# tuffy/flac-codec

Hardware: AMD Instinct MI355X
Metric: Msamples/s encode at level 8, 48kHz/24-bit stereo; bit-exact vs reference (higher is better)
Workload: dtype i32/i64 (+f64 LPC analysis); 1 GPU; config 3: 48 kHz/24-bit stereo, blocksize 4096, level 8 (Options::best: LPC order 12, partition order 6, mid-side, exhaustive); 8192 frames per GPU per step, PCM resident in HBM, frame bytes produc...; level=L8, frames_per_gpu=8192, contexts=3, parallelism=frame ranges x1

## Files before the change

flac-codec_amd/csrc/autocorr.hip:

```cpp
#include "kernels/types.h"

#include <stdlib.h>

#include <type_traits>

namespace {
#include "kernels/common.inc"
#include "kernels/lpc.inc"
#include "kernels/autocorr.inc"

template <int NL, bool STEREO>
bool launch_autocorr3(const Params &p, uint32_t frame0, uint32_t nframes, uint32_t n, const double *win, hipStream_t st) {
    const uint32_t groups = (nframes * p.ncand + 63) / 64;
    if constexpr (STEREO) {
        if (p.inter) {
            if (groups <= 64 && NL == 13)
                hipLaunchKernelGGL(HIP_KERNEL_NAME(k_autocorr4<13, 8, true, true, 0, true>), dim3(groups), dim3(512), 0, st, p,
                                   frame0, nframes, n, win);
            else
                hipLaunchKernelGGL(HIP_KERNEL_NAME(k_autocorr4<NL, 4, true, true, 0, true>), dim3(groups), dim3(256), 0, st, p,
                                   frame0, nframes, n, win);
            return true;
        }
    }
    if constexpr (!STEREO) {
        if (p.split_src) {
#define AC4_SPLIT(C)                                                                                                      \
    hipLaunchKernelGGL(HIP_KERNEL_NAME(k_autocorr4<NL, 4, false, true, C, true>), dim3(groups), dim3(256), 0, st, p, frame0, \
                       nframes, n, win)
            if (p.channels == 8) AC4_SPLIT(8);
            else if (p.channels == 4) AC4_SPLIT(4);
            else AC4_SPLIT(0);
#undef AC4_SPLIT
            return true;
        }
    }
    if (p.ac_split == 2)
        hipLaunchKernelGGL(HIP_KERNEL_NAME(k_autocorr4<NL, 2, STEREO>), dim3(groups), dim3(128), 0, st, p,
                           frame0, nframes, n, win);
    else
        hipLaunchKernelGGL(HIP_KERNEL_NAME(k_autocorr4<NL, 4, STEREO>), dim3(groups), dim3(256), 0, st, p,
                           frame0, nframes, n, win);
    return false;
}
template <bool STEREO>
bool launch_autocorr3_nl(const Params &p, uint32_t frame0, uint32_t nframes, uint32_t n, const double *win, hipStream_t st) {
    const uint32_t nl = p.max_lpc_order + 1;
    if (nl <= 5) return launch_autocorr3<5, STEREO>(p, frame0, nframes, n, win, st);
    if (nl <= 9) return launch_autocorr3<9, STEREO>(p, frame0, nframes, n, win, st);
    if (nl <= 13) return launch_autocorr3<13, STEREO>(p, frame0, nframes, n, win, st);
    return launch_autocorr3<17, STEREO>(p, frame0, nframes, n, win, st);
}
bool try_autocorr3(const Params &p, uint32_t frame0, uint32_t nframes, uint32_t n, const double *win, hipStream_t st,
                   bool *fused) {
    *fused = false;
    if (n < 32 || n % 32 != 0) return false;
    const bool stereo = p.stereo4 && p.ncand == 4 && p.channels == 2 && p.bps <= 24;
    const bool indep = !p.stereo4 && p.ncand == p.channels;
    if (!stereo && !indep) return false;
    if (p.max_lpc_order > 16) {
        if (n % 64 != 0) return false;
        const uint32_t groups = (nframes * p.ncand + 63) / 64;
        if (stereo && p.inter) {
            hipLaunchKernelGGL(HIP_KERNEL_NAME(k_autocorr4_deep<true, true>), dim3(groups), dim3(256), 0, st, p, frame0,
                               nframes, n, win);
        } else if (stereo) {
            hipLaunchKernelGGL(HIP_KERNEL_NAME(k_autocorr4_deep<true>), dim3(groups), dim3(256), 0, st, p, frame0,
                               nframes, n, win);
// ... 61 lines not shown
```

flac-codec_amd/csrc/flacenc_gpu.hip:

```cpp
#include "kernels/types.h"
#include "kernels/place_rule.h"
#include "batch_route.h"
#include "lpc_host.h"
#include "ragged_plan.h"

#include <ctype.h>
#include <math.h>
#include <stdint.h>
#include <stdio.h>
#include <stdlib.h>
#include <string.h>

#include <algorithm>
#include <atomic>
#include <cmath>
#include <chrono>
#include <functional>
#include <mutex>
#include <thread>
#include <string>
#include <type_traits>
#include <vector>

thread_local std::string g_last_error;

static std::atomic<uint64_t> g_early_downloads{0}, g_early_remainders{0};
extern "C" void flacgpu_early_download_counters(uint64_t *queued, uint64_t *with_remainder) {
    if (queued) *queued = g_early_downloads.load();
    if (with_remainder) *with_remainder = g_early_remainders.load();
}
static constexpr uint32_t kDeferMargin16 = 48;
static constexpr uint32_t kDeferWords = DEFER_SLOTS * DEFER_SLOT_WORDS;
static constexpr uint32_t kTurnWords = 4;
Knobs read_knobs() {
    Knobs k;
    auto on = [](const char *name) { return getenv(name) != nullptr; };
    k.no_direct = on("FLACGPU_NO_DIRECT");
    k.no_cand_pair = on("FLACGPU_NO_CAND_PAIR");
    k.force_fir_check = on("FLACGPU_FIR_CHECK");
    k.no_xpose = on("FLACGPU_NO_XPOSE");
    k.no_ac_fma = on("FLACGPU_NO_AC_FMA");
    k.no_hand = on("FLACGPU_NO_HAND");
    k.no_direct_short = on("FLACGPU_NO_DIRECT_SHORT");
    k.no_ragged = on("FLACGPU_NO_RAGGED");
    k.no_w64 = on("FLACGPU_NO_W64");
    k.no_fused_pack = on("FLACGPU_NO_FUSED_PACK");
    k.no_frame64 = on("FLACGPU_NO_FRAME64");
    k.early_download = on("FLACGPU_EARLY_DOWNLOAD");
    if (const char *e = getenv("FLACGPU_CAND_GRID")) k.cand_grid = (uint32_t)atoi(e);
    if (const char *e = getenv("FLACGPU_DEFER_FIXED")) k.defer_fixed = atoi(e);
    if (const char *e = getenv("FLACGPU_DEFER_MARGIN16")) k.defer_margin16 = atoi(e);
    const char *t = getenv("FLACGPU_TEST_KNOBS");
    if (t && t[0] == '1') {
        k.experiment_mfma_ac = on("FLACGPU_EXPERIMENT_MFMA_AC");
        if (const char *e = getenv("FLACGPU_TIE_BAND")) { k.has_tie_band = true; k.tie_band = atof(e); }
        if (const char *e = getenv("FLACGPU_TIE_PERTURB")) { k.has_tie_perturb = true; k.tie_perturb = atof(e); }
        if (const char *e = getenv("FLACGPU_FIR_SUSPECT_BITS")) k.fir_suspect_bits = (uint32_t)atoi(e);
    }
    return k;
}

namespace {
#include "kernels/common.inc"
#include "kernels/k0_split.inc"
#include "kernels/generic_analysis.inc"
#include "kernels/generic_fir.inc"
#include "kernels/decide_emit.inc"
}
using namespace flacgpu_k;
using flacenc_route::Route;
using flacenc_route::RouteBatch;
using flacenc_route::RouteContext;

struct flacgpu_ctx;
static uint32_t *defer_stats_of(const flacgpu_ctx *c);
static int ctx_sync(flacgpu_ctx *c);
static hipStream_t ctx_stream(flacgpu_ctx *c);

struct flacgpu_ctx {
    flacgpu_options opts;
    uint32_t bps, channels, max_frames, ldb, ncand, stereo4;
    int device;
    int32_t *d_in = nullptr, *d_planar = nullptr, *d_resid = nullptr;
    double *d_window_full = nullptr, *d_window_last = nullptr, *d_log2_thr = nullptr, *d_ac = nullptr;
    CandInfo *d_cinfo = nullptr;
    SubPlan *d_fixed = nullptr, *d_cand = nullptr, *d_out = nullptr;
    LpcParams *d_lpc = nullptr;
    FrameInfo *d_finfo = nullptr;
    uint32_t *d_hand = nullptr;
    flacgpu_frame_plan *d_fplan = nullptr;
    uint32_t *d_stats_base = nullptr;
    uint32_t *d_stats = nullptr;
    uint32_t *d_orbits = nullptr;
    uint32_t *d_ties = nullptr;
    double tie_band = 1e-9, tie_perturb = 0.0;
    Knobs knobs;
    uint64_t *d_seg_fn = nullptr, *h_seg = nullptr;
    const int32_t **d_seg_ptr = nullptr;
    std::vector<flacgpu_segment> segs;
    bool seg_pending = false;
    bool seg_active = false;
    bool seg_direct = false;
    uint32_t *d_rag_tab = nullptr, *h_rag_tab = nullptr;
    PlaceRun *d_rag_runs = nullptr, *h_rag_runs = nullptr;
    double *d_rag_pool = nullptr;
    uint64_t rag_pool_cap = 0;
    std::vector<std::pair<uint32_t, uint32_t>> rag_pool_at;
    std::vector<double> rag_pool_host;
    uint64_t rag_pool_uploads = 0;
    std::vector<uint32_t> rag_n;
// ... 599 lines not shown
        } else {
            begin_plain_batch(c);
        }
    }
    const uint32_t B = c->opts.block_size;
    const bool ragged = c->rag_active;
    if (!ragged)
    for (uint32_t n : {n_frames > 1 ? B : last_len, last_len}) {
        uint32_t tz = (uint32_t)__builtin_ctz(n);
        if ((tz < c->opts.max_partition_order ? tz : c->opts.max_partition_order) > (uint32_t)MAXP) {
            g_last_error = "effective partition order > 6: the reference panics (MAX_PARTITIONS = 64)";
            return FLACGPU_ERR_UNSUPPORTED;
        }
    }
    if (!ragged && last_len != B && last_len != c->window_last_len) {
        if (int rc = upload_window(c, last_len, c->d_window_last, st)) return rc;
        c->window_last_len = last_len;
    }
    Params p;
    fill_params(c, n_frames, last_len, p);
    if (ragged) {
        p.frame_n = c->d_rag_tab;
        p.frame_win = c->d_rag_tab + c->max_frames;
        p.window_pool = c->d_rag_pool;
    }
    c->host_out = nullptr;
    c->out_in_host = false;

    int evi = 0;
    for (auto &u : c->ev_used) u = false;
    auto mark = [&](int k) {
        if (c->timing) {
            (void)hipEventRecord(c->ev[evi], st);
            c->ev_used[k] = true;
            evi++;
        }
    };
    int order_of_marks[FLACGPU_N_KERNELS];
    int n_marks = 0;
    auto begin = [&](int k) {
        order_of_marks[n_marks++] = k;
        mark(k);
    };

    const Route r = given ? *given : route_of(c, aligned16(d_pcm), layout, n_frames, last_len, packed_bytes);
    const uint32_t ncb = n_frames * c->ncand;
    const bool ranged = c->rng_cnt != 0;
    const uint32_t rf0 = ranged ? c->rng_f0 : 0u, rcnt = ranged ? c->rng_cnt : n_frames;
    const bool first_range = rf0 == 0;
    if (first_range) HIP_TRY(hipMemsetAsync(c->d_stats_base, 0, sizeof(uint32_t) * (kTurnWords + 4 + (size_t)ncb), st));
    const bool direct = r.input == Route::DIRECT_STEREO, xpose = r.input == Route::SPLIT_XPOSE;
    const bool split = r.input == Route::SPLIT || xpose;
    if (direct) p.inter = d_pcm;
    if (r.hand) p.hand_meta = c->d_hand;
    if (r.segments_in_place) p.inter_tab = c->d_seg_ptr;
    if (split) {
        p.split_src = d_pcm;
        p.split_dst = (c->channels == 1 || xpose) ? nullptr : c->d_planar;
        p.xpose = xpose ? 1u : 0u;
        if (c->channels == 1) p.planar = d_pcm;
    }
    c->abs_valid = false;
    if (c->d_abs && first_range) HIP_TRY(hipMemsetAsync(c->d_abs, 0, sizeof(unsigned long long) * 4 * n_frames, st));
    if (!r.in_place()) begin(0);
    bool have_orbits = true;
    if (r.input == Route::K0_PACKED) {
        launch_k0_packed(c, packed_bytes, n_frames, last_len, st);
    } else if (r.input == Route::PLANAR_IN_PLACE) {
        p.planar = d_pcm;
        have_orbits = false;
    } else if (r.input == Route::K0_COPY) {
        have_orbits = launch_k0(c, d_pcm, layout, n_frames, last_len, 0, n_frames, st);
    }
    if (!have_orbits)
        launch_orbits(p, c->d_orbits, st);
    const size_t dyn2 = (2 * (size_t)B + B / 16 + 16) * sizeof(int32_t);
    if (c->stereo4 && !p.exhaustive && !c->abs_valid && !(direct && p.max_lpc_order == 0)) {
        begin(1);
        if (direct) hipLaunchKernelGGL(k_stereo_stats_t<true>, dim3(n_frames), dim3(WG), 0, st, p);
        else hipLaunchKernelGGL(k_stereo_stats_t<false>, dim3(n_frames), dim3(WG), 0, st, p);
    }
    if (!r.in_place())
        hipLaunchKernelGGL(k_candinfo, dim3((ncb + WG - 1) / WG), dim3(WG), 0, st, p, c->d_orbits,
                           c->abs_valid ? c->d_abs : nullptr);
    Params pf = p, pg = p;
    pf.f0 = rf0;
    pf.fcount = ranged ? rcnt : r.fast_analysis;
    pg.f0 = r.fast_analysis;
    pg.fcount = n_frames - r.fast_analysis;
    const bool lpc = p.max_lpc_order > 0;
    const bool fork = lpc && !c->timing && pg.fcount != 0;
    hipStream_t sf = fork ? c->aux_stream : st;
    if (fork) {
        HIP_TRY(hipEventRecord(c->ev_fork, st));
        HIP_TRY(hipStreamWaitEvent(sf, c->ev_fork, 0));
    }
    if (pg.fcount) {
        begin(2);
        if (B > LDS_BLOCK_LIMIT) hipLaunchKernelGGL(k_fixed_t<true>, dim3(pg.fcount * c->ncand), dim3(WG), 0, sf, pg);
        else hipLaunchKernelGGL(k_fixed_t<false>, dim3(pg.fcount * c->ncand), dim3(WG), dyn2, sf, pg);
    }
    if (fork) HIP_TRY(hipEventRecord(c->ev_join, sf));
    if (lpc) {
        const uint32_t H = ((p.max_lpc_order + 1) + 3u) & ~3u;
        begin(3);
        const uint32_t full = ragged ? 0u : (last_len == B) ? n_frames : n_frames - 1;
// ... 1282 lines not shown
```

flac-codec_amd/csrc/host/batch_route.cpp:

```cpp
#include "batch_route.h"

#include <stddef.h>

namespace flacenc_route {

RouteContext route_context(uint32_t channels, uint32_t bps, uint32_t block_size, uint32_t max_lpc_order,
                           uint32_t max_partition_order, bool exhaustive, const Knobs &knobs) {
    RouteContext c;
    c.channels = channels;
    c.bps = bps;
    c.block_size = block_size;
    c.max_lpc_order = max_lpc_order;
    c.max_partition_order = max_partition_order;
    c.exhaustive = exhaustive;
    c.stereo4 = (channels == 2 && bps < 32) ? 1u : 0u;
    c.ncand = c.stereo4 ? 4u : channels;
    c.has_hand = c.stereo4 && block_size == FN && max_lpc_order > 0 && !knobs.no_hand;
    c.has_edges = channels >= 5;
    c.knobs = knobs;
    return c;
}

namespace {
constexpr int kInterleaved = 0, kPlanar = 1;
constexpr size_t kFrameLdsBytes = 150 * 1024;
bool fits_lds(uint32_t fb_words) { return (size_t)fb_words * sizeof(int32_t) <= kFrameLdsBytes; }
}

Route plan_route(const RouteContext &c, const RouteBatch &b) {
    Route r;
    if (b.ragged) return r;
    const Knobs &kn = c.knobs;
    const uint32_t B = c.block_size, C_ = c.channels, n_frames = b.n_frames;
    const bool whole_blocks = b.last_len == B;
    const uint32_t full = whole_blocks ? n_frames : n_frames - 1;
    const bool narrow = c.bps + (c.stereo4 ? 1u : 0u) <= 25u;
    const bool po_ok = c.max_partition_order <= (uint32_t)MAXP;
    const uint32_t fbw_any = frame_fb_words(C_, c.bps, B);

    const bool w64 = narrow && wave_block_size(B) && (c.max_lpc_order <= 16 || B == FN) && po_ok && !kn.no_w64;
    r.fast_analysis = w64 ? full : 0;

    const uint32_t fbw = (c.stereo4 && c.exhaustive && frame_fb_words_exhaustive_stereo(c.bps, B) < fbw_any)
                             ? frame_fb_words_exhaustive_stereo(c.bps, B) : fbw_any;
    const bool f64w = narrow && wave_block_size(B) && (c.max_lpc_order <= 16 || (B == FN && C_ <= 4)) && (C_ <= 4 || B == FN) &&
                      po_ok && fits_lds(fbw) && !kn.no_fused_pack && !kn.no_frame64;
    r.fast_pack = f64w ? full : 0;
    r.host_out_possible = r.fast_pack != 0 && r.fast_pack == n_frames;
    const bool all_fast = whole_blocks && w64 && f64w;

    const bool in_place_ok = !b.packed_bytes && b.aligned16 && whole_blocks && po_ok && c.lag_split != 2 &&
                             !(kn.no_direct || kn.no_w64 || kn.experiment_mfma_ac);
    const bool direct = in_place_ok && b.layout == kInterleaved && c.stereo4 && C_ == 2 && c.bps <= 24 &&
                        (B == FN || (wave_block_size(B) && c.max_lpc_order <= 16 && !kn.no_direct_short)) &&
                        !kn.no_fused_pack && !kn.no_frame64 && fits_lds(fbw_any);
    const bool planar_rows = !b.packed_bytes && b.aligned16 && (b.layout == kPlanar || C_ == 1) && (B % 4 == 0) && whole_blocks &&
                             !kn.no_direct;
    const bool split = in_place_ok && !c.stereo4 && c.ncand == C_ && c.max_lpc_order >= 1 && c.max_lpc_order <= 16 && B == FN &&
                       c.bps <= 25u && (C_ == 1 ? planar_rows : b.layout == kInterleaved);
    const bool xpose = split && all_fast && !kn.no_xpose && c.bps >= 8 &&
                       (C_ == 3 || C_ == 4 || ((C_ == 8 || C_ == 6) && c.has_edges));
    r.input = direct ? Route::DIRECT_STEREO
              : split ? (xpose ? Route::SPLIT_XPOSE : Route::SPLIT)
              : b.packed_bytes ? Route::K0_PACKED
              : planar_rows ? Route::PLANAR_IN_PLACE
                            : Route::K0_COPY;
    r.hand = direct && B == FN && c.max_lpc_order > 0 && c.has_hand;
    r.segments_in_place = b.segments_in_place_wanted && r.in_place() && C_ >= 2;
    r.k4_in_autocorr = r.in_place() && c.max_lpc_order >= 1 && c.max_lpc_order <= 16;

    if (!b.whole_call || b.packed_bytes || c.timing) return r;
    if (c.two_ranges && n_frames >= 256 && all_fast && fits_lds(fbw_any) && (b.layout == kInterleaved || b.layout == kPlanar)) {
        r.two_ranges = true;
        r.input = (b.layout == kPlanar && planar_rows) ? Route::PLANAR_IN_PLACE : Route::K0_COPY;
        r.hand = r.k4_in_autocorr = r.segments_in_place = false;
        return r;
    }
    if (c.chunk_samples && B == FN && C_ >= 2 && r.in_place() && all_fast && r.k4_in_autocorr &&
        (c.stereo4 ? c.exhaustive : !c.chunk_auto)) {
        const uint32_t chunk = (uint32_t)(c.chunk_samples / ((uint64_t)B * C_)) & ~63u;
        if (chunk >= 256 && n_frames >= chunk + chunk / 2) r.range_frames = chunk;
    }
    return r;
}

}

extern "C" void flacenc_plan_route_row(const int32_t *in, uint32_t *out) {
    using namespace flacenc_route;
    Knobs kn;
    const uint32_t bits = (uint32_t)in[14];
    kn.no_direct = bits & 1u;
    kn.no_w64 = bits & 2u;
    kn.no_fused_pack = bits & 4u;
    kn.no_frame64 = bits & 8u;
    kn.no_direct_short = bits & 16u;
    kn.no_xpose = bits & 32u;
    kn.no_hand = bits & 64u;
    kn.experiment_mfma_ac = bits & 128u;
    RouteContext c = route_context((uint32_t)in[0], (uint32_t)in[1], (uint32_t)in[2], (uint32_t)in[3], (uint32_t)in[4], in[5] != 0, kn);
    c.lag_split = in[11];
    c.timing = in[12] != 0;
    if (in[15] >= 0) {
        c.chunk_samples = chunk_samples_of(in[15]);
        c.chunk_auto = false;
    }
    c.two_ranges = in[16] != 0;
    RouteBatch b;
    b.layout = in[6];
    b.aligned16 = in[7] != 0;
    b.last_len = (uint32_t)in[8];
    b.n_frames = (uint32_t)in[9];
    b.packed_bytes = (uint32_t)in[10];
    b.segments_in_place_wanted = in[13] != 0;
    b.whole_call = in[17] != 0;
    const Route r = plan_route(c, b);
    out[0] = (uint32_t)r.input;
    out[1] = r.hand;
    out[2] = r.fast_analysis;
    out[3] = r.fast_pack;
    out[4] = r.k4_in_autocorr;
    out[5] = r.range_frames;
    out[6] = r.two_ranges;
    out[7] = r.host_out_possible;
    out[8] = r.segments_in_place;
}
```

flac-codec_amd/csrc/host/batch_route.h:

```cpp
#ifndef FLACENC_HOST_BATCH_ROUTE_H
#define FLACENC_HOST_BATCH_ROUTE_H
#include <stdint.h>

#include "../kernels/shape.h"

namespace flacenc_route {

struct RouteContext {
    uint32_t channels = 0, bps = 0, block_size = 0, max_lpc_order = 0, max_partition_order = 0;
    bool exhaustive = false;
    uint32_t stereo4 = 0, ncand = 0;
    bool has_hand = false;
    bool has_edges = false;
    Knobs knobs;
    int lag_split = 4;
    bool two_ranges = false;
    uint32_t chunk_samples = 64u << 20;
    bool chunk_auto = true;
    bool timing = false;
};
inline uint32_t chunk_samples_of(int msamples) { return msamples <= 0 ? 0u : (uint32_t)(msamples < 2047 ? msamples : 2047) << 20; }
RouteContext route_context(uint32_t channels, uint32_t bps, uint32_t block_size, uint32_t max_lpc_order,
                           uint32_t max_partition_order, bool exhaustive, const Knobs &knobs);

struct RouteBatch {
    uint32_t n_frames = 0, last_len = 0;
    int layout = 0;
    bool aligned16 = false;
    uint32_t packed_bytes = 0;
    bool segments_in_place_wanted = false;
    bool whole_call = false;
    bool ragged = false;
};

struct Route {
    enum Input {
        K0_COPY,
        K0_PACKED,
        PLANAR_IN_PLACE,
        DIRECT_STEREO,
        SPLIT,
        SPLIT_XPOSE
    } input = K0_COPY;
    bool hand = false;
    uint32_t fast_analysis = 0;
    uint32_t fast_pack = 0;
    bool k4_in_autocorr = false;
    uint32_t range_frames = 0;
    bool two_ranges = false;
    bool host_out_possible = false;
    bool segments_in_place = false;

    bool in_place() const { return input == DIRECT_STEREO || input == SPLIT || input == SPLIT_XPOSE; }
};

Route plan_route(const RouteContext &c, const RouteBatch &b);

}
#endif
```

flac-codec_amd/csrc/kernels/autocorr.inc:

```


__device__ __forceinline__ void ac4_progress_prio(uint32_t t, uint32_t ntiles) {
    if ((t & 7u) == 0) {
        const uint32_t qd = 4u * t / ntiles;
        if (qd == 0) __builtin_amdgcn_s_setprio(3);
        else if (qd == 1) __builtin_amdgcn_s_setprio(2);
        else if (qd == 2) __builtin_amdgcn_s_setprio(1);
        else __builtin_amdgcn_s_setprio(0);
    }
}

template <int A, int LG, bool FIRST, bool FMA = false>
__device__ __forceinline__ void ac3_block(const double (&w)[16], const double (&prev)[16],
                                          double (&acc)[LG]) {
    if constexpr (FMA) {
        static_assert(!FIRST, "the first block of a frame lies under the window's taper");
#pragma unroll
        for (int s = 0; s < 16; s++) {
#pragma unroll
            for (int k = 0; k < LG; k++) {
                const int lag = A + k;
                const double o = (s - lag >= 0) ? w[(s - lag >= 0) ? s - lag : 0]
                                                : prev[(s - lag >= 0) ? 0 : 16 + s - lag];
                acc[k] = __builtin_fma(w[s], o, acc[k]);
// ... 33 lines not shown
#pragma unroll
            for (int k = 0; k < LG; k++) {
                const int idx = s - (A + k);
                const double o = idx >= 0 ? w[idx >= 0 ? idx : 0]
                               : idx >= -16 ? p1[(idx < 0 && idx >= -16) ? 16 + idx : 0]
                                            : p2[(idx < -16) ? 32 + idx : 0];
                acc[k] = __builtin_fma(w[s], o, acc[k]);
            }
            __builtin_amdgcn_sched_barrier(0);
        }
        return;
    }
#pragma unroll
    for (int s = 0; s < 16; s++) {
        double prod[LG];
#pragma unroll
        for (int k = 0; k < LG; k++) {
            const int idx = s - (A + k);
            const double o = idx >= 0 ? w[idx >= 0 ? idx : 0]
                           : idx >= -16 ? p1[(idx < 0 && idx >= -16) ? 16 + idx : 0]
                                        : p2[(idx < -16) ? 32 + idx : 0];
            prod[k] = w[s] * o;
        }
        __builtin_amdgcn_sched_barrier(0);
#pragma unroll
        for (int k = 0; k < LG; k++) {
            const int lag = A + k;
            if (FIRST == 1 && s < lag) continue;
            if (FIRST == 2 && 16 + s < lag) continue;
            acc[k] = acc[k] + prod[k];
        }
        __builtin_amdgcn_sched_barrier(0);
    }
}

constexpr int AC4_TS = 32;
constexpr int AC4_LDW = AC4_TS + 2;

__device__ __forceinline__ int32_t dpp_row_ror8(int32_t v) {
    int32_t r = __builtin_amdgcn_update_dpp(0, v, 0x128, 0xf, 0xf, false);
    asm volatile("" : "+v"(r));
    return r;
}

template <bool STEREO>
struct Ac4Units {
    static constexpr int PER_TILE = STEREO ? 8 : 16;
    static constexpr int COST = STEREO ? 20 : 10;
};
struct Ac4Share {
    int units[8], first[8];
};
template <bool STEREO>
constexpr Ac4Share ac4_share_n(int ns, const int (&lg)[8]) {
    Ac4Share r{};
    int cost[8] = {};
    for (int w = 0; w < 8; w++) {
        cost[w] = 64 * lg[w];
        r.units[w] = 0;
    }
    for (int u = 0; u < Ac4Units<STEREO>::PER_TILE; u++) {
        int best = 0;
        for (int w = 1; w < ns; w++)
            if (cost[w] < cost[best]) best = w;
        r.units[best]++;
        cost[best] += Ac4Units<STEREO>::COST;
    }
    int f = 0;
    for (int w = 0; w < 8; w++) {
        r.first[w] = f;
        f += r.units[w];
    }
    return r;
}
template <bool STEREO>
constexpr Ac4Share ac4_share(int ns, int lg0, int lg1, int lg2, int lg3) {
    const int lg[8] = {lg0, lg1, lg2, lg3, 0, 0, 0, 0};
    return ac4_share_n<STEREO>(ns, lg);
}

template <int U, bool STEREO>
struct Ac4Producer {
    static constexpr int NU = U > 0 ? U : 1;
    const int32_t *gsrc[NU];
    const double *wsrc[NU];
    uint32_t dst_a[NU], dst_b[NU];
    uint32_t sh_a[NU], sh_b[NU];
    int32_t sgn;
    uint32_t ntiles;
    int2 stage[NU];
    double2 wst[NU];
};

template <int U, int U0, bool STEREO>
__device__ __forceinline__ void ac4_setup(const Params &p, uint32_t frame0, uint32_t nframes, uint32_t n,
                                          const double *__restrict__ win, uint32_t group,
                                          Ac4Producer<U, STEREO> &P) {
    const uint32_t lane = threadIdx.x & 63;
    const uint32_t total = nframes * p.ncand;
    const uint32_t cand0 = group * 64;
    P.ntiles = n / AC4_TS;
    auto wasted_of = [&](uint32_t cc) -> uint32_t {
        const CandInfo ci = p.cinfo[(size_t)frame0 * p.ncand + (cc < total ? cc : total - 1)];
        return (ci.active && !ci.is_const) ? ci.wasted : 0u;
    };
    if constexpr (STEREO) {
        const uint32_t f_lo = cand0 / 4, f_last = nframes - 1;
        const uint32_t is_r = (lane >> 3) & 1u;
        P.sgn = is_r ? -1 : 1;
#pragma unroll
        for (int it = 0; it < U; it++) {
// ... 41 lines not shown
        const double w[2] = {P.wst[it].x, P.wst[it].y};
        const int32_t own[2] = {P.stage[it].x, P.stage[it].y};
        double a[2], b[2];
#pragma unroll
        for (int e = 0; e < 2; e++) {
            a[e] = (double)(own[e] >> P.sh_a[it]) * w[e];
            if constexpr (STEREO) {
                const int32_t other = dpp_row_ror8(own[e]);
                const int32_t v = __mul24(own[e], P.sgn) + other;
                b[e] = (double)(v >> P.sh_b[it]) * w[e];
            }
        }
        *reinterpret_cast<double2 *>(dst + P.dst_a[it]) = make_double2(a[0], a[1]);
        if constexpr (STEREO) *reinterpret_cast<double2 *>(dst + P.dst_b[it]) = make_double2(b[0], b[1]);
    }
}
template <int U>
struct Ac4Direct {
    static constexpr int NU = U > 0 ? U : 1;
    const int32_t *gsrc[NU];
    const double *wsrc[NU];
    uint32_t dst[NU];
    uint32_t orow[NU];
    uint32_t ors[NU][4];
    uint32_t ntiles;
    int2 stage[NU];
    double wst[NU];
};
template <int U, int U0>
__device__ __forceinline__ void ac4_setup_direct(const Params &p, uint32_t frame0, uint32_t nframes, uint32_t n,
                                                 const double *__restrict__ win, uint32_t group, Ac4Direct<U> &P) {
    const uint32_t lane = threadIdx.x & 63;
    const uint32_t f_lo = group * 16, f_last = nframes - 1;
    P.ntiles = n / AC4_TS;
#pragma unroll
    for (int it = 0; it < U; it++) {
        const uint32_t u = U0 + it;
        const uint32_t col = 16u * (u & 1u) + (lane & 15u);
        const uint32_t fl = 4u * (u >> 1) + (lane >> 4);
        const uint32_t fr = f_lo + fl < nframes ? f_lo + fl : f_last;
        P.gsrc[it] = inter_frame(p, frame0 + fr, 2 * n) + (size_t)col * 2;
        P.wsrc[it] = win + col;
        P.dst[it] = (4 * fl) * AC4_LDW + col;
        P.orow[it] = 4 * fl;
#pragma unroll
        for (int c = 0; c < 4; c++) P.ors[it][c] = 0;
    }
}
template <int U>
__device__ __forceinline__ void ac4_fetch(Ac4Direct<U> &P, uint32_t t) {
    t = t < P.ntiles ? t : P.ntiles - 1;
#pragma unroll
    for (int it = 0; it < U; it++) {
        P.stage[it] = *reinterpret_cast<const int2 *>(P.gsrc[it] + t * (AC4_TS * 2));
        P.wst[it] = P.wsrc[it][t * AC4_TS];
    }
}
template <int U>
__device__ __forceinline__ void ac4_convert(Ac4Direct<U> &P, double *dst, bool = false) {
#pragma unroll
    for (int it = 0; it < U; it++) {
        const int32_t l = P.stage[it].x, r = P.stage[it].y;
        const int32_t m = (l + r) >> 1, sd = l - r;
        const double w = P.wst[it];
        P.ors[it][0] |= (uint32_t)l;
        P.ors[it][1] |= (uint32_t)r;
        P.ors[it][2] |= (uint32_t)m;
        P.ors[it][3] |= (uint32_t)sd;
        double *d = dst + P.dst[it];
        d[0] = (double)l * w;
        d[AC4_LDW] = (double)r * w;
        d[2 * AC4_LDW] = (double)m * w;
        d[3 * AC4_LDW] = (double)sd * w;
    }
}
template <int U>
__device__ __forceinline__ void ac4_finish(const Ac4Direct<U> &P, uint32_t *ors) {
#pragma unroll
    for (int it = 0; it < U; it++) {
#pragma unroll
        for (int c = 0; c < 4; c++) {
            uint32_t v = P.ors[it][c];
#pragma unroll
            for (int off = 8; off > 0; off >>= 1) v |= __shfl_xor(v, off, 64);
            if ((threadIdx.x & 15) == 0) atomicOr(&ors[P.orow[it] + c], v);
        }
    }
}
template <int U>
struct Ac4Split {
    static constexpr int NU = U > 0 ? U : 1;
    const int32_t *gsrc[NU];
    int32_t *pdst[NU];
    const double *wsrc[NU];
    uint32_t dst[NU], orow[NU], ors[NU];
    uint32_t ntiles, stride;
    bool store;
    int2 stage[NU];
    double2 wst[NU];
};
template <int U, int U0>
__device__ __forceinline__ void ac4_setup_split(const Params &p, uint32_t frame0, uint32_t nframes, uint32_t n,
                                                const double *__restrict__ win, uint32_t group, Ac4Split<U> &P) {
    const uint32_t lane = threadIdx.x & 63;
    const uint32_t total = nframes * p.ncand, cand0 = group * 64, C = p.channels;
    P.ntiles = n / AC4_TS;
    P.stride = C;
// ... 164 lines not shown
#pragma unroll
    for (int s = 0; s < 16; s++) w1[s] = 0.0;
    ac4_fetch(P, 0);
    convert(wt[0], 0);
    ac4_fetch(P, 1);
    __syncthreads();
    auto tile = [&](auto first, uint32_t t) {
        constexpr bool FIRST = decltype(first)::value;
        ac4_progress_prio(t, P.ntiles);
        const double *cur = wt[t & 1] + myrow;
        ac4_read(cur, 0, w0);
        __builtin_amdgcn_sched_barrier(0);
        convert(wt[(t + 1) & 1], t + 1);
        ac4_fetch(P, t + 2);
        __builtin_amdgcn_sched_barrier(0);
        const bool exact = !FIRST && t >= p.fma_t0 && t < p.fma_t1;
        if (exact) {
            if constexpr (!FIRST) ac3_block<A, LG, false, true>(w0, w1, acc);
        } else {
            ac3_block<A, LG, FIRST>(w0, w1, acc);
        }
        ac4_read(cur, 16, w1);
        __builtin_amdgcn_sched_barrier(0);
        if (exact) ac3_block<A, LG, false, true>(w1, w0, acc);
        else ac3_block<A, LG, false>(w1, w0, acc);
        __syncthreads();
    };
    tile(std::true_type{}, 0);
#pragma unroll 1
    for (uint32_t t = 1; t < P.ntiles; t++) tile(std::false_type{}, t);
    if constexpr (DIRECT) {
        ac4_finish(P, ors);
        __syncthreads();
        const uint32_t orv = ors[lane];
        if (A == 0 && live) p.stats[4 + (size_t)frame0 * p.ncand + cc] = orv;
        const uint32_t w2 = orv ? 2u * (uint32_t)__builtin_ctz(orv) : 0u;
        const double scale = __longlong_as_double((long long)(1023u - w2) << 52);
#pragma unroll
        for (int k = 0; k < LG; k++) acc[k] *= scale;
    }
    if (live) {
        double *out = p.ac + ((size_t)frame0 * p.ncand + cc) * AC_LD + A;
#pragma unroll
        for (int k = 0; k < LG; k++) out[k] = acc[k];
    }
    if constexpr (FUSE_LPC) {
        static_assert(DIRECT, "the tile loop and the OR exchange end with barriers: wt[0] is idle here");
        double *row = wt[0] + lane * AC4_LDW + A;
#pragma unroll
        for (int k = 0; k < LG; k++) row[k] = acc[k];
    }
}

template <int NL, int NS, bool STEREO, bool DIRECT = false, int SPLITC = 0, bool FUSE_LPC = false>
__global__ void __launch_bounds__(64 * NS)
k_autocorr4(Params p, uint32_t frame0, uint32_t nframes, uint32_t n, const double *__restrict__ win) {
    __shared__ __attribute__((aligned(16))) double wt[2][64 * AC4_LDW];
    __shared__ uint32_t ors[64];
    const uint32_t wave = __builtin_amdgcn_readfirstlane(threadIdx.x >> 6);
    constexpr int B0 = 0, B1 = NL * 1 / NS, B2 = NL * 2 / NS, B3 = NL * 3 / NS, B4 = NL * 4 / NS;
    if constexpr (NS == 8) {
        constexpr int C0 = 0, C1 = NL * 1 / 8, C2 = NL * 2 / 8, C3 = NL * 3 / 8, C4 = NL * 4 / 8, C5 = NL * 5 / 8,
                      C6 = NL * 6 / 8, C7 = NL * 7 / 8, C8 = NL;
        constexpr int LGS[8] = {C1 - C0, C2 - C1, C3 - C2, C4 - C3, C5 - C4, C6 - C5, C7 - C6, C8 - C7};
        constexpr Ac4Share S = ac4_share_n<STEREO>(8, LGS);
#define AC4_W(i, a, b) case i: ac4_wave<a, b - a, S.units[i], S.first[i], STEREO, DIRECT, 0, FUSE_LPC>(p, wt, frame0, nframes, n, win, blockIdx.x, ors); break;
        switch (wave) {
            AC4_W(0, C0, C1) AC4_W(1, C1, C2) AC4_W(2, C2, C3) AC4_W(3, C3, C4) AC4_W(4, C4, C5) AC4_W(5, C5, C6) AC4_W(6, C6, C7)
            default: ac4_wave<C7, C8 - C7, S.units[7], S.first[7], STEREO, DIRECT, 0, FUSE_LPC>(p, wt, frame0, nframes, n, win, blockIdx.x, ors); break;
        }
#undef AC4_W
    } else if constexpr (NS == 2) {
        constexpr Ac4Share S = ac4_share<STEREO>(2, B1 - B0, B2 - B1, 0, 0);
        if (wave == 0) ac4_wave<B0, B1 - B0, S.units[0], S.first[0], STEREO, DIRECT>(p, wt, frame0, nframes, n, win, blockIdx.x, ors);
        else ac4_wave<B1, B2 - B1, S.units[1], S.first[1], STEREO, DIRECT>(p, wt, frame0, nframes, n, win, blockIdx.x, ors);
    } else {
        constexpr Ac4Share S = ac4_share<STEREO>(4, B1 - B0, B2 - B1, B3 - B2, B4 - B3);
        switch (wave) {
        case 0: ac4_wave<B0, B1 - B0, S.units[0], S.first[0], STEREO, DIRECT, SPLITC, FUSE_LPC>(p, wt, frame0, nframes, n, win, blockIdx.x, ors); break;
        case 1: ac4_wave<B1, B2 - B1, S.units[1], S.first[1], STEREO, DIRECT, SPLITC, FUSE_LPC>(p, wt, frame0, nframes, n, win, blockIdx.x, ors); break;
        case 2: ac4_wave<B2, B3 - B2, S.units[2], S.first[2], STEREO, DIRECT, SPLITC, FUSE_LPC>(p, wt, frame0, nframes, n, win, blockIdx.x, ors); break;
        default: ac4_wave<B3, B4 - B3, S.units[3], S.first[3], STEREO, DIRECT, SPLITC, FUSE_LPC>(p, wt, frame0, nframes, n, win, blockIdx.x, ors); break;
        }
    }
    if constexpr (FUSE_LPC) {
        static_assert(NS != 2 && NL - 1 <= 16, "DIRECT instantiations: four or eight lag-group waves, order <= 16");
        __syncthreads();
        if (wave != 0) return;
        const uint32_t lane = threadIdx.x;
        const uint32_t cc = blockIdx.x * 64 + lane;
        if (cc >= nframes * p.ncand) return;
        const uint32_t idx = frame0 * p.ncand + cc;
        const bool act = p.exhaustive ? true : active_in_assignment(p.finfo[idx / p.ncand].assignment, idx % p.ncand);
        const CandInfo ci = cand_info_from_or(p, idx % p.ncand, ors[lane], act);
        p.cinfo[idx] = ci;
        const double *row = wt[0] + lane * AC4_LDW;
        lpc_candidate<NL - 1>(p, idx, n, ci, [row](int i) { return row[i]; });
    }
}

template <int A, int LG, int U, int U0, bool STEREO, bool DIRECT = false>
__device__ __forceinline__ void ac4_wave_deep(const Params &p, double (*wt)[64 * AC4_LDW], uint32_t frame0,
                                              uint32_t nframes, uint32_t n, const double *__restrict__ win,
                                              uint32_t group, uint32_t *ors = nullptr) {
    const uint32_t lane = threadIdx.x & 63;
    std::conditional_t<DIRECT, Ac4Direct<U>, Ac4Producer<U, STEREO>> P;
    if constexpr (DIRECT) {
        ac4_setup_direct<U, U0>(p, frame0, nframes, n, win, group, P);
        if (threadIdx.x < 64) ors[threadIdx.x] = 0;
    } else {
        ac4_setup<U, U0, STEREO>(p, frame0, nframes, n, win, group, P);
    }
    const uint32_t total = nframes * p.ncand;
    const uint32_t cc = group * 64 + lane;
    const bool live = cc < total;
    double acc[LG];
#pragma unroll
    for (int k = 0; k < LG; k++) acc[k] = -0.0;
    double wa[16], wb[16], wc[16], wd[16];
#pragma unroll
    for (int s = 0; s < 16; s++) wc[s] = wd[s] = 0.0;
    ac4_fetch(P, 0);
    ac4_convert(P, wt[0]);
    ac4_fetch(P, 1);
    __syncthreads();
    const uint32_t myrow = lane * AC4_LDW;
    auto tile = [&](auto first, uint32_t t, double (&X0)[16], double (&X1)[16], double (&Y0)[16], double (&Y1)[16]) {
        constexpr bool FIRST = decltype(first)::value;
        ac4_progress_prio(t, P.ntiles);
        const double *cur = wt[t & 1] + myrow;
        ac4_read(cur, 0, X0);
        __builtin_amdgcn_sched_barrier(0);
        if constexpr (DIRECT) ac4_convert(P, wt[(t + 1) & 1], t + 1 >= p.fma_t0 && t + 1 < p.fma_t1);
        else ac4_convert(P, wt[(t + 1) & 1]);
        ac4_fetch(P, t + 2);
        __builtin_amdgcn_sched_barrier(0);
        const bool exact = !FIRST && t >= p.fma_t0 && t < p.fma_t1;
        if (exact) {
            if constexpr (!FIRST) ac3_block_deep<A, LG, 0, true>(X0, Y1, Y0, acc);
// ... 378 lines not shown
```

flac-codec_amd/csrc/kernels/shape.h:

```cpp
#ifndef FLACGPU_KERNEL_SHAPE_H
#define FLACGPU_KERNEL_SHAPE_H
#include <stdint.h>

#ifdef __HIPCC__
#define FLACGPU_HD __host__ __device__
#else
#define FLACGPU_HD
#endif

constexpr int MAXP = 6;
constexpr uint32_t FN = 4096;

constexpr uint32_t LDS_BLOCK_LIMIT = 16384;

FLACGPU_HD constexpr uint32_t frame_fb_words(uint32_t channels, uint32_t bps, uint32_t n = FN) {
    return (((16u + 2u) * 8u + channels * (n * (bps + 1u) + 64u) + 31u) / 32u + 2u + 3u) & ~3u;
}

FLACGPU_HD constexpr uint32_t frame_fb_words_exhaustive_stereo(uint32_t bps, uint32_t n = FN) {
    return (((16u + 2u) * 8u + 2u * (n * bps + 64u) + 31u) / 32u + 2u + 3u) & ~3u;
}

#define FLACGPU_WAVE_SIZES(X) X(4096, 64) X(2304, 36) X(2048, 32) X(1152, 18) X(1024, 16)
inline bool wave_block_size(uint32_t B) {
    switch (B) {
#define X(n, spl) case n:
        FLACGPU_WAVE_SIZES(X)
#undef X
        return true;
    default: return false;
    }
}

struct Knobs {
    bool no_direct = false, no_w64 = false, no_fused_pack = false, no_frame64 = false,
         early_download = false,
         no_hand = false,
         no_direct_short = false,
         no_ac_fma = false,
         no_xpose = false,
         no_cand_pair = false,
         no_ragged = false;
    bool force_fir_check = false;
    uint32_t cand_grid = 0;
    bool experiment_mfma_ac = false;
    bool has_tie_band = false, has_tie_perturb = false;
    double tie_band = 0.0, tie_perturb = 0.0;
    uint32_t fir_suspect_bits = 0;
    int defer_fixed = -1;
    int defer_margin16 = -1;
};
#endif
```

flac-codec_amd/csrc/kernels/types.h:

```cpp
#ifndef FLACGPU_KERNEL_TYPES_H
#define FLACGPU_KERNEL_TYPES_H
#include <hip/hip_runtime.h>

#include <stdint.h>

#include <string>
#include <type_traits>

#include "flacenc_gpu.h"
#include "shape.h"


constexpr int WG = 256;
constexpr int NLEAF = 1 << MAXP;
constexpr int NNODE = 2 * NLEAF - 1;

extern thread_local std::string g_last_error;

#define HIP_TRY(expr)                                                                   \
    do {                                                                                \
        hipError_t e_ = (expr);                                                         \
        if (e_ != hipSuccess) {                                                         \
            g_last_error = std::string(#expr) + ": " + hipGetErrorString(e_);           \
            return FLACGPU_ERR_HIP;                                                     \
        }                                                                               \
    } while (0)

struct DeviceGuard {
    int prev = -1;
    bool changed = false;
    explicit DeviceGuard(int dev) {
        if (hipGetDevice(&prev) == hipSuccess && prev != dev) changed = hipSetDevice(dev) == hipSuccess;
    }
    ~DeviceGuard() { if (changed) (void)hipSetDevice(prev); }
    DeviceGuard(const DeviceGuard &) = delete;
    DeviceGuard &operator=(const DeviceGuard &) = delete;
};

typedef flacgpu_subframe_plan SubPlan;

struct CandInfo {
    uint8_t active;
    uint8_t wasted;
    uint8_t bps;
    uint8_t is_const;
};

struct LpcParams {
    int32_t status;
    uint8_t order, precision, shift;
    uint8_t est8;
    int32_t qlp[FLACGPU_MAX_LPC_ORDER];
};

struct FrameInfo {
    uint8_t assignment;
    uint8_t pad[3];
};

struct Params {
    uint32_t channels, bps, block_size, ldb;
    uint32_t ncand;
    uint32_t stereo4;
    uint32_t mid_side, exhaustive;
    uint32_t max_lpc_order, max_po, use_rice2;
    uint32_t n_frames, last_len;
    uint32_t f0, fcount;
    uint32_t ac_split;
    uint32_t fma_t0, fma_t1;
    const int32_t *planar;
    const int32_t *inter;
    const int32_t *const *inter_tab;
    const int32_t *split_src;
    int32_t *split_dst;
    uint32_t xpose;
    const double *window_full, *window_last;
    const double *log2_thr;
    CandInfo *cinfo;
    SubPlan *fixed_plan, *cand_plan, *out_plan;
    LpcParams *lpc;
    double *ac;
    FrameInfo *finfo;
    flacgpu_frame_plan *frame_plan;
    int32_t *residuals;
    uint32_t *stats;
    int32_t *big_scratch;
    uint32_t big_stride;
    uint32_t *tie_list;
    uint32_t tie_cap;
    double tie_band, tie_perturb;
    uint32_t check_fir;
    uint32_t fir_suspect_bits;
    uint32_t defer_fixed, defer_margin16;
    uint32_t *defer_stats;
    uint32_t *turn_counter;
    uint32_t *hand_meta;
    const uint32_t *frame_n;
    const uint32_t *frame_win;
    const double *window_pool;
};


__device__ __forceinline__ const int32_t *inter_frame(const Params &p, uint32_t frame, uint32_t frame_dwords) {
    return p.inter_tab ? p.inter_tab[frame] : p.inter + (size_t)frame * frame_dwords;
}
__device__ __forceinline__ const int32_t *split_frame(const Params &p, uint32_t frame, uint32_t frame_dwords) {
    return p.inter_tab ? p.inter_tab[frame] : p.split_src + (size_t)frame * frame_dwords;
}

__host__ __device__ constexpr uint32_t big_scratch_ints(uint32_t block_size) {
    return 2u * (block_size + block_size / 16u + 16u) + 64u;
}
constexpr uint32_t DEFER_SLOTS = 64, DEFER_SLOT_WORDS = 16;
constexpr int AC_LD = 36;

struct PackParams {
    uint64_t first_frame_number;
    const uint64_t *frame_numbers = nullptr;
    uint32_t sample_rate;
    uint32_t *out_words;
    uint64_t *frame_off;
// ... 66 lines not shown
```

Baseline: 196,800 Msamples/s.

## Add opt-in two-wave stereo autocorrelation kernel with block-ahead prefetch

Adds a two-wave variant of the fused interleaved-stereo autocorrelation kernel for LPC order up to 12. Each wave takes half of the lags and uses a register block-ahead routine that loads the next 16 windowed samples while it accumulates. The variant is chosen through a new route field and env/bit knobs, but the default still selects four waves, so it only runs when asked for. The tile fetch now reads through an explicit global-address-space 64-bit load, which may let the compiler emit a global rather than a flat load.

```diff
diff --git a/flac-codec_amd/csrc/autocorr.hip b/flac-codec_amd/csrc/autocorr.hip
--- a/flac-codec_amd/csrc/autocorr.hip
+++ b/flac-codec_amd/csrc/autocorr.hip
@@ -14,6 +14,13 @@
     const uint32_t groups = (nframes * p.ncand + 63) / 64;
     if constexpr (STEREO) {
         if (p.inter) {
+            if constexpr (NL <= 13) {
+                if (p.ac_waves == 2) {
+                    hipLaunchKernelGGL(HIP_KERNEL_NAME(k_autocorr4<NL, 2, true, true, 0, true>), dim3(groups), dim3(128), 0, st, p,
+                                       frame0, nframes, n, win);
+                    return true;
+                }
+            }
             if (groups <= 64 && NL == 13)
                 hipLaunchKernelGGL(HIP_KERNEL_NAME(k_autocorr4<13, 8, true, true, 0, true>), dim3(groups), dim3(512), 0, st, p,
                                    frame0, nframes, n, win);
diff --git a/flac-codec_amd/csrc/flacenc_gpu.hip b/flac-codec_amd/csrc/flacenc_gpu.hip
--- a/flac-codec_amd/csrc/flacenc_gpu.hip
+++ b/flac-codec_amd/csrc/flacenc_gpu.hip
@@ -56,6 +56,7 @@
         if (const char *e = getenv("FLACGPU_TIE_BAND")) { k.has_tie_band = true; k.tie_band = atof(e); }
         if (const char *e = getenv("FLACGPU_TIE_PERTURB")) { k.has_tie_perturb = true; k.tie_perturb = atof(e); }
         if (const char *e = getenv("FLACGPU_FIR_SUSPECT_BITS")) k.fir_suspect_bits = (uint32_t)atoi(e);
+        if (const char *e = getenv("FLACGPU_AC_WAVES2")) k.ac_waves2 = atoi(e) != 0 ? 1 : 0;
     }
     return k;
 }
@@ -761,6 +762,7 @@
     const bool direct = r.input == Route::DIRECT_STEREO, xpose = r.input == Route::SPLIT_XPOSE;
     const bool split = r.input == Route::SPLIT || xpose;
     if (direct) p.inter = d_pcm;
+    p.ac_waves = r.ac_waves;
     if (r.hand) p.hand_meta = c->d_hand;
     if (r.segments_in_place) p.inter_tab = c->d_seg_ptr;
     if (split) {
diff --git a/flac-codec_amd/csrc/host/batch_route.cpp b/flac-codec_amd/csrc/host/batch_route.cpp
--- a/flac-codec_amd/csrc/host/batch_route.cpp
+++ b/flac-codec_amd/csrc/host/batch_route.cpp
@@ -25,6 +25,7 @@
 constexpr int kInterleaved = 0, kPlanar = 1;
 constexpr size_t kFrameLdsBytes = 150 * 1024;
 bool fits_lds(uint32_t fb_words) { return (size_t)fb_words * sizeof(int32_t) <= kFrameLdsBytes; }
+constexpr uint32_t kAcWavesDefault = 4;
 }
 
 Route plan_route(const RouteContext &c, const RouteBatch &b) {
@@ -68,12 +69,15 @@
     r.hand = direct && B == FN && c.max_lpc_order > 0 && c.has_hand;
     r.segments_in_place = b.segments_in_place_wanted && r.in_place() && C_ >= 2;
     r.k4_in_autocorr = r.in_place() && c.max_lpc_order >= 1 && c.max_lpc_order <= 16;
+    if (direct && r.k4_in_autocorr && B == FN && c.max_lpc_order <= 12)
+        r.ac_waves = kn.ac_waves2 < 0 ? kAcWavesDefault : kn.ac_waves2 ? 2u : 4u;
 
     if (!b.whole_call || b.packed_bytes || c.timing) return r;
     if (c.two_ranges && n_frames >= 256 && all_fast && fits_lds(fbw_any) && (b.layout == kInterleaved || b.layout == kPlanar)) {
         r.two_ranges = true;
         r.input = (b.layout == kPlanar && planar_rows) ? Route::PLANAR_IN_PLACE : Route::K0_COPY;
         r.hand = r.k4_in_autocorr = r.segments_in_place = false;
+        r.ac_waves = 0;
         return r;
     }
     if (c.chunk_samples && B == FN && C_ >= 2 && r.in_place() && all_fast && r.k4_in_autocorr &&
@@ -86,7 +90,7 @@
 
 }
 
-extern "C" void flacenc_plan_route_row(const int32_t *in, uint32_t *out) {
+static flacenc_route::Route route_of_row(const int32_t *in) {
     using namespace flacenc_route;
     Knobs kn;
     const uint32_t bits = (uint32_t)in[14];
@@ -98,6 +102,8 @@
     kn.no_xpose = bits & 32u;
     kn.no_hand = bits & 64u;
     kn.experiment_mfma_ac = bits & 128u;
+    if (bits & 256u) kn.ac_waves2 = 1;
+    if (bits & 512u) kn.ac_waves2 = 0;
     RouteContext c = route_context((uint32_t)in[0], (uint32_t)in[1], (uint32_t)in[2], (uint32_t)in[3], (uint32_t)in[4], in[5] != 0, kn);
     c.lag_split = in[11];
     c.timing = in[12] != 0;
@@ -114,7 +120,10 @@
     b.packed_bytes = (uint32_t)in[10];
     b.segments_in_place_wanted = in[13] != 0;
     b.whole_call = in[17] != 0;
-    const Route r = plan_route(c, b);
+    return plan_route(c, b);
+}
+extern "C" void flacenc_plan_route_row(const int32_t *in, uint32_t *out) {
+    const flacenc_route::Route r = route_of_row(in);
     out[0] = (uint32_t)r.input;
     out[1] = r.hand;
     out[2] = r.fast_analysis;
@@ -125,3 +134,5 @@
     out[7] = r.host_out_possible;
     out[8] = r.segments_in_place;
 }
+extern "C" uint32_t flacenc_plan_route_ac_waves(const int32_t *in) { return route_of_row(in).ac_waves; }
+extern "C" uint32_t flacenc_route_ac_waves_default(void) { return flacenc_route::kAcWavesDefault; }
diff --git a/flac-codec_amd/csrc/host/batch_route.h b/flac-codec_amd/csrc/host/batch_route.h
--- a/flac-codec_amd/csrc/host/batch_route.h
+++ b/flac-codec_amd/csrc/host/batch_route.h
@@ -46,6 +46,7 @@
     uint32_t fast_analysis = 0;
     uint32_t fast_pack = 0;
     bool k4_in_autocorr = false;
+    uint32_t ac_waves = 0;
     uint32_t range_frames = 0;
     bool two_ranges = false;
     bool host_out_possible = false;
diff --git a/flac-codec_amd/csrc/kernels/autocorr.inc b/flac-codec_amd/csrc/kernels/autocorr.inc
--- a/flac-codec_amd/csrc/kernels/autocorr.inc
+++ b/flac-codec_amd/csrc/kernels/autocorr.inc
@@ -109,11 +109,11 @@
     int units[8], first[8];
 };
 template <bool STEREO>
-constexpr Ac4Share ac4_share_n(int ns, const int (&lg)[8]) {
+constexpr Ac4Share ac4_share_n(int ns, const int (&lg)[8], int lag_cost = 64) {
     Ac4Share r{};
     int cost[8] = {};
     for (int w = 0; w < 8; w++) {
-        cost[w] = 64 * lg[w];
+        cost[w] = lag_cost * lg[w];
         r.units[w] = 0;
     }
     for (int u = 0; u < Ac4Units<STEREO>::PER_TILE; u++) {
@@ -261,7 +261,9 @@
     t = t < P.ntiles ? t : P.ntiles - 1;
 #pragma unroll
     for (int it = 0; it < U; it++) {
-        P.stage[it] = *reinterpret_cast<const int2 *>(P.gsrc[it] + t * (AC4_TS * 2));
+        typedef const __attribute__((address_space(1))) unsigned long long global_u64;
+        const unsigned long long lr = *(global_u64 *)(uintptr_t)(P.gsrc[it] + t * (AC4_TS * 2));
+        P.stage[it] = make_int2((int32_t)(uint32_t)lr, (int32_t)(uint32_t)(lr >> 32));
         P.wst[it] = P.wsrc[it][t * AC4_TS];
     }
 }
@@ -532,6 +534,119 @@
     }
 }
 
+template <int A, int LG, bool FIRST, bool FMA>
+__device__ __forceinline__ void ac3_block_ahead(const double (&w)[16], double (&prev)[16], double (&acc)[LG],
+                                                const double *next) {
+    constexpr int MAXLAG = A + LG - 1;
+    static_assert(MAXLAG <= 15, "the last read must find its pair of history samples dead inside the block");
+    static_assert(!(FIRST && FMA), "the first block of a frame lies under the window's taper");
+    double nx[16];
+#pragma unroll
+    for (int s = 0; s < 16; s++) {
+#pragma unroll
+        for (int q = 0; q < 8; q++) {
+            const int at = 2 * q + MAXLAG - 14 > 0 ? 2 * q + MAXLAG - 14 : 0;
+            if (at == s) {
+                const double2 v = *reinterpret_cast<const double2 *>(next + 2 * q);
+                nx[2 * q] = v.x;
+                nx[2 * q + 1] = v.y;
+            }
+        }
+        __builtin_amdgcn_sched_barrier(0);
+        if constexpr (FMA) {
+#pragma unroll
+            for (int k = 0; k < LG; k++) {
+                const int lag = A + k;
+                const double o = (s - lag >= 0) ? w[(s - lag >= 0) ? s - lag : 0]
+                                                : prev[(s - lag >= 0) ? 0 : 16 + s - lag];
+                acc[k] = __builtin_fma(w[s], o, acc[k]);
+            }
+            __builtin_amdgcn_sched_barrier(0);
+        } else {
+            double prod[LG];
+#pragma unroll
+            for (int k = 0; k < LG; k++) {
+                const int lag = A + k;
+                const double o = (s - lag >= 0) ? w[(s - lag >= 0) ? s - lag : 0]
+                                                : prev[(s - lag >= 0) ? 0 : 16 + s - lag];
+                prod[k] = w[s] * o;
+            }
+            __builtin_amdgcn_sched_barrier(0);
+#pragma unroll
+            for (int k = 0; k < LG; k++) {
+                const int lag = A + k;
+                if (FIRST && s < lag) continue;
+                acc[k] = acc[k] + prod[k];
+            }
+            __builtin_amdgcn_sched_barrier(0);
+        }
+    }
+#pragma unroll
+    for (int s = 0; s < 16; s++) prev[s] = nx[s];
+}
+
+template <int A, int LG, int U, int U0>
+__device__ __forceinline__ void ac4_wave2(const Params &p, double (*wt)[64 * AC4_LDW], uint32_t frame0, uint32_t nframes,
+                                          uint32_t n, const double *__restrict__ win, uint32_t group, uint32_t *ors) {
+    const uint32_t lane = threadIdx.x & 63;
+    Ac4Direct<U> P;
+    ac4_setup_direct<U, U0>(p, frame0, nframes, n, win, group, P);
+    if (threadIdx.x < 64) ors[threadIdx.x] = 0;
+    const uint32_t total = nframes * p.ncand;
+    const uint32_t cc = group * 64 + lane;
+    const bool live = cc < total;
+    double acc[LG];
+#pragma unroll
+    for (int k = 0; k < LG; k++) acc[k] = -0.0;
+    const uint32_t myrow = lane * AC4_LDW;
+    double w0[16], w1[16];
+#pragma unroll
+    for (int s = 0; s < 16; s++) w1[s] = 0.0;
+    ac4_fetch(P, 0);
+    ac4_convert(P, wt[0]);
+    ac4_fetch(P, 1);
+    __syncthreads();
+    ac4_read(wt[0] + myrow, 0, w0);
+    auto tile = [&](auto first, auto fma, uint32_t t) {
+        constexpr bool FIRST = decltype(first)::value, FMA = decltype(fma)::value;
+        ac4_progress_prio(t, P.ntiles);
+        const double *cur = wt[t & 1] + myrow, *nxt = wt[(t + 1) & 1] + myrow;
+        ac4_convert(P, wt[(t + 1) & 1]);
+        ac4_fetch(P, t + 2);
+        __builtin_amdgcn_sched_barrier(0);
+        ac3_block_ahead<A, LG, FIRST, FMA>(w0, w1, acc, cur + 16);
+        __syncthreads();
+        ac3_block_ahead<A, LG, false, FMA>(w1, w0, acc, nxt);
+    };
+    const uint32_t nt = P.ntiles;
+    const uint32_t ta = p.fma_t0 < 1 ? 1 : p.fma_t0 < nt ? p.fma_t0 : nt;
+    const uint32_t tb = p.fma_t1 < ta ? ta : p.fma_t1 < nt ? p.fma_t1 : nt;
+    tile(std::true_type{}, std::false_type{}, 0);
+    uint32_t t = 1;
+#pragma unroll 1
+    for (; t < ta; t++) tile(std::false_type{}, std::false_type{}, t);
+#pragma unroll 1
+    for (; t < tb; t++) tile(std::false_type{}, std::true_type{}, t);
+#pragma unroll 1
+    for (; t < nt; t++) tile(std::false_type{}, std::false_type{}, t);
+    ac4_finish(P, ors);
+    __syncthreads();
+    const uint32_t orv = ors[lane];
+    if (A == 0 && live) p.stats[4 + (size_t)frame0 * p.ncand + cc] = orv;
+    const uint32_t w2 = orv ? 2u * (uint32_t)__builtin_ctz(orv) : 0u;
+    const double scale = __longlong_as_double((long long)(1023u - w2) << 52);
+#pragma unroll
+    for (int k = 0; k < LG; k++) acc[k] *= scale;
+    if (live) {
+        double *out = p.ac + ((size_t)frame0 * p.ncand + cc) * AC_LD + A;
+#pragma unroll
+        for (int k = 0; k < LG; k++) out[k] = acc[k];
+    }
+    double *row = wt[0] + lane * AC4_LDW + A;
+#pragma unroll
+    for (int k = 0; k < LG; k++) row[k] = acc[k];
+}
+
 template <int NL, int NS, bool STEREO, bool DIRECT = false, int SPLITC = 0, bool FUSE_LPC = false>
 __global__ void __launch_bounds__(64 * NS)
 k_autocorr4(Params p, uint32_t frame0, uint32_t nframes, uint32_t n, const double *__restrict__ win) {
@@ -550,6 +665,13 @@
             default: ac4_wave<C7, C8 - C7, S.units[7], S.first[7], STEREO, DIRECT, 0, FUSE_LPC>(p, wt, frame0, nframes, n, win, blockIdx.x, ors); break;
         }
 #undef AC4_W
+    } else if constexpr (NS == 2 && FUSE_LPC) {
+        static_assert(STEREO && DIRECT && SPLITC == 0, "two lag-group waves with K4 in the tail: interleaved stereo only");
+        constexpr int H0 = (NL + 1) / 2;
+        constexpr int LGS[8] = {H0, NL - H0, 0, 0, 0, 0, 0, 0};
+        constexpr Ac4Share S = ac4_share_n<true>(2, LGS, 48);
+        if (wave == 0) ac4_wave2<0, H0, S.units[0], S.first[0]>(p, wt, frame0, nframes, n, win, blockIdx.x, ors);
+        else ac4_wave2<H0, NL - H0, S.units[1], S.first[1]>(p, wt, frame0, nframes, n, win, blockIdx.x, ors);
     } else if constexpr (NS == 2) {
         constexpr Ac4Share S = ac4_share<STEREO>(2, B1 - B0, B2 - B1, 0, 0);
         if (wave == 0) ac4_wave<B0, B1 - B0, S.units[0], S.first[0], STEREO, DIRECT>(p, wt, frame0, nframes, n, win, blockIdx.x, ors);
@@ -564,7 +686,7 @@
         }
     }
     if constexpr (FUSE_LPC) {
-        static_assert(NS != 2 && NL - 1 <= 16, "DIRECT instantiations: four or eight lag-group waves, order <= 16");
+        static_assert(NL - 1 <= 16, "DIRECT instantiations: order <= 16");
         __syncthreads();
         if (wave != 0) return;
         const uint32_t lane = threadIdx.x;
diff --git a/flac-codec_amd/csrc/kernels/shape.h b/flac-codec_amd/csrc/kernels/shape.h
--- a/flac-codec_amd/csrc/kernels/shape.h
+++ b/flac-codec_amd/csrc/kernels/shape.h
@@ -47,6 +47,7 @@
     bool has_tie_band = false, has_tie_perturb = false;
     double tie_band = 0.0, tie_perturb = 0.0;
     uint32_t fir_suspect_bits = 0;
+    int ac_waves2 = -1;
     int defer_fixed = -1;
     int defer_margin16 = -1;
 };
diff --git a/flac-codec_amd/csrc/kernels/types.h b/flac-codec_amd/csrc/kernels/types.h
--- a/flac-codec_amd/csrc/kernels/types.h
+++ b/flac-codec_amd/csrc/kernels/types.h
@@ -67,6 +67,7 @@
     uint32_t n_frames, last_len;
     uint32_t f0, fcount;
     uint32_t ac_split;
+    uint32_t ac_waves;
     uint32_t fma_t0, fma_t1;
     const int32_t *planar;
     const int32_t *inter;
```

Result: no change. 198,600 Msamples/s, median of 6 (+0.9%).
